# haoheliu/voicefixer

Measured on AMD Instinct MI355X. Metric: seconds-of-44.1kHz-audio restored per wall-second, higher is better.
Workload: dtype f32

## Files before the change

voicefixer_amd/csrc/vfx_conv.hip:

```cpp
#include "vfx_common.h"
#include <cstdio>
#include <cstdlib>
#include <cstring>
#include <map>
#include <mutex>
#include <string>
#include <type_traits>
#include <vector>

#ifndef VFX_X3_ABL
#define VFX_X3_ABL 0
#endif
#ifndef VFX_ABL
#define VFX_ABL 0
#endif
#define VFX_MAXPH 8
#define VFX_MAXT 9

typedef float f32x16 __attribute__((ext_vector_type(16)));
typedef unsigned int u32x4 __attribute__((ext_vector_type(4)));

#if VFX_ABL & 8
__device__ unsigned long long g_dbg[10];
__device__ unsigned long long g_dbgx[6];
// ... 906 lines not shown
        static const bool dump = VFX_DEV_ENV("VFX_DEBUG_ARGS") && atoi(VFX_DEV_ENV("VFX_DEBUG_ARGS")) != 0;
        if (dump) {
            fprintf(stderr, "conv table:");
            const unsigned* w = reinterpret_cast<const unsigned*>(&tb);
            for (size_t i = 0; i < sizeof(PhaseTab) / 4; ++i) fprintf(stderr, " %08x", w[i]);
            fprintf(stderr, "\n");
        }
    }
    ConvTables* d = nullptr;
    if (hipMalloc((void**)&d, sizeof(ConvTables)) != hipSuccess) return nullptr;
    if (hipMemcpy(d, &tb, sizeof(ConvTables), hipMemcpyHostToDevice) != hipSuccess) return nullptr;
    cache.emplace(std::move(key), d);
    return d;
}

static thread_local int g_last_tile = 0;
extern "C" int vfx_last_conv_tile(void) { return g_last_tile; }

static inline int floor4(int v) { return v >= 0 ? (v & ~3) : -(((-v) + 3) & ~3); }

template <int BM, int BL, int WGM, int WGL, int KC, bool FAST, int NXV = 4, bool SPLITK = false>
static int launch_one(const ConvArgs& a, dim3 grid, size_t lds, hipStream_t s) {
    static unsigned long long attr_set = 0;
    int attr_dev = 0;
    if (hipGetDevice(&attr_dev) != hipSuccess) attr_dev = 0;
    auto kern = conv_taps_kernel<BM, BL, WGM, WGL, KC, FAST, NXV, SPLITK>;
    if (!((attr_set >> (attr_dev & 63)) & 1ull)) {
        hipError_t e = hipFuncSetAttribute(reinterpret_cast<const void*>(kern),
                                           hipFuncAttributeMaxDynamicSharedMemorySize, 160 * 1024);
        if (e != hipSuccess) return (int)e;
        attr_set |= 1ull << (attr_dev & 63);
    }
    {
        static const bool dump = VFX_DEV_ENV("VFX_DEBUG_ARGS") && atoi(VFX_DEV_ENV("VFX_DEBUG_ARGS")) != 0;
        if (dump) {
            fprintf(stderr, "conv_taps<%d,%d,%d,%d,%d,%d,%d,%d> grid %u %u %u lds %zu args:", BM, BL, WGM, WGL, KC, (int)FAST,
                    NXV, (int)SPLITK, grid.x, grid.y, grid.z, lds);
            const unsigned* w = reinterpret_cast<const unsigned*>(&a);
            for (size_t i = 0; i < sizeof(ConvArgs) / 4; ++i) fprintf(stderr, " %08x", w[i]);
            fprintf(stderr, "\n");
        }
    }
    hipLaunchKernelGGL(kern, grid, dim3(64 * WGM * WGL), lds, s, a);
    VFX_LAUNCHED();
    return vfx_last_error();
}

template <int BM, int BL, int WGM, int WGL, int KC>
static int launch_cfg(const ConvArgs& a, int ntiles, int gy, int gz, size_t lds, hipStream_t s) {
    const int nfast = a.tile_hi - a.tile_lo;
    int rc = VFX_OK;
    if (a.ksplit > 1) {
        if (nfast > 0) rc = launch_one<BM, BL, WGM, WGL, KC, true, 4, true>(a, dim3(nfast, gy, gz), lds, s);
        if (rc == VFX_OK && ntiles - nfast > 0)
            rc = launch_one<BM, BL, WGM, WGL, KC, false, 4, true>(a, dim3(ntiles - nfast, gy, gz), lds, s);
        return rc;
    }
    if (nfast > 0) {
        const dim3 grid((nfast + a.tpw - 1) / a.tpw, gy, gz);
        if constexpr (WGM * WGL == 4) {
            rc = a.nxv <= 1   ? launch_one<BM, BL, WGM, WGL, KC, true, 1>(a, grid, lds, s)
                 : a.nxv == 2 ? launch_one<BM, BL, WGM, WGL, KC, true, 2>(a, grid, lds, s)
                 : a.nxv == 3 ? launch_one<BM, BL, WGM, WGL, KC, true, 3>(a, grid, lds, s)
                              : launch_one<BM, BL, WGM, WGL, KC, true, 4>(a, grid, lds, s);
        } else {
            rc = launch_one<BM, BL, WGM, WGL, KC, true, 4>(a, grid, lds, s);
        }
    }
    if (rc == VFX_OK && ntiles - nfast > 0)
        rc = launch_one<BM, BL, WGM, WGL, KC, false>(a, dim3(ntiles - nfast, gy, gz), lds, s);
    return rc;
}

static int fill_segments(ConvArgs& a, ConvTables& tb, int nphase, const PhaseSpec* phs, int BL, int KC,
                         bool exact = false) {
    int segw = 0;
    bool halo[VFX_MAXPH];
    for (int p = 0; p < nphase; ++p) {
        int mn = phs[p].taps[0].off, mx = mn;
        for (int t = 1; t < phs[p].ntaps; ++t) {
            mn = phs[p].taps[t].off < mn ? phs[p].taps[t].off : mn;
            mx = phs[p].taps[t].off > mx ? phs[p].taps[t].off : mx;
        }
        const int span = mx - mn;
        halo[p] = (long long)BL + span + 3 <= (long long)phs[p].ntaps * (BL + 3);
        int need;
        if (halo[p]) {
            need = exact ? BL : (mn - floor4(mn)) + BL + span;
        } else {
            need = exact ? BL : BL + 3;
        }
        need = (need + 3) & ~3;
        segw = need > segw ? need : segw;
    }
    a.segw = segw;
    int xs = 0;
    for (int p = 0; p < nphase; ++p) {
        PhaseTab& T = tb.ph[p];
        T.ntaps = phs[p].ntaps;
        T.ooff = phs[p].ooff;
        if (halo[p]) {
            int mn = phs[p].taps[0].off;
            for (int t = 1; t < phs[p].ntaps; ++t) mn = phs[p].taps[t].off < mn ? phs[p].taps[t].off : mn;
            const int org = exact ? mn : floor4(mn);
            T.nseg = 1;
            T.seg_org[0] = org;
            for (int t = 0; t < phs[p].ntaps; ++t) {
                T.tap_lds[t] = phs[p].taps[t].off - org;
                T.tap_w[t] = phs[p].taps[t].slab;
            }
        } else {
            T.nseg = phs[p].ntaps;
            for (int t = 0; t < phs[p].ntaps; ++t) {
                const int org = exact ? phs[p].taps[t].off : floor4(phs[p].taps[t].off);
                T.seg_org[t] = org;
                T.tap_lds[t] = t * KC * segw + (phs[p].taps[t].off - org);
                T.tap_w[t] = phs[p].taps[t].slab;
            }
        }
        const int fl = T.nseg * KC * segw;
        xs = fl > xs ? fl : xs;
    }
    a.xs_floats = xs;
    return VFX_OK;
}



static float* splitk_workspace(hipStream_t s, size_t bytes) {
    static std::mutex mu;
    static std::map<std::pair<int, hipStream_t>, std::pair<float*, size_t>> pool;
    int dev = 0;
    if (hipGetDevice(&dev) != hipSuccess) return nullptr;
    std::lock_guard<std::mutex> lock(mu);
    auto& e = pool[std::make_pair(dev, s)];
    if (e.second < bytes) {
        static std::vector<float*> retired;
        if (e.first) retired.push_back(e.first);
        e.first = nullptr;
        e.second = 0;
        const size_t want = bytes + bytes / 2;
        if (hipMalloc((void**)&e.first, want) != hipSuccess) { e.first = nullptr; return nullptr; }
        e.second = want;
    }
    return e.first;
}


#include "vfx_convw.inc"
#include "vfx_convwg.inc"
#include "vfx_convwg4p.inc"
#include "vfx_convwg4x.inc"
#include "vfx_convtw.inc"
#include "vfx_convwg2d.inc"
#include "vfx_resblk4.inc"
#include "vfx_resblk4s.inc"
#include "vfx_convh.inc"

template <int BM, int BL, int WGM, int WGL, int NT, int MODE, int ROWS = 1>
static int launch_x3_one(const ConvArgs& a, dim3 grid, size_t lds, hipStream_t s) {
    static unsigned long long attr_set = 0;
    int attr_dev = 0;
    if (hipGetDevice(&attr_dev) != hipSuccess) attr_dev = 0;
    auto kern = conv_x3_kernel<BM, BL, WGM, WGL, NT, MODE, ROWS>;
    if (!((attr_set >> (attr_dev & 63)) & 1ull)) {
        hipError_t e = hipFuncSetAttribute(reinterpret_cast<const void*>(kern),
                                           hipFuncAttributeMaxDynamicSharedMemorySize, 160 * 1024);
        if (e != hipSuccess) return (int)e;
        attr_set |= 1ull << (attr_dev & 63);
    }
    hipLaunchKernelGGL(kern, grid, dim3(256), lds, s, a);
    VFX_LAUNCHED();
    return vfx_last_error();
}

template <int BM, int BL, int WGM, int WGL>
static int launch_x3_tile(const ConvArgs& a, int nt, int mode, int rows, dim3 grid, size_t lds, hipStream_t s) {
    if (rows == 3 && nt == 3) return launch_x3_one<BM, BL, WGM, WGL, 3, 0, 3>(a, grid, lds, s);
    if (rows == 3) return launch_x3_one<BM, BL, WGM, WGL, 1, 0, 3>(a, grid, lds, s);
#define VFX_X3(NT_)                                                                                  \
    if (nt == NT_)                                                                                   \
        return mode == 2   ? launch_x3_one<BM, BL, WGM, WGL, NT_, 2>(a, grid, lds, s)                \
               : mode == 1 ? launch_x3_one<BM, BL, WGM, WGL, NT_, 1>(a, grid, lds, s)                \
                           : launch_x3_one<BM, BL, WGM, WGL, NT_, 0>(a, grid, lds, s);
    VFX_X3(1)
    VFX_X3(2)
    VFX_X3(3)
#undef VFX_X3
    return VFX_ENOTSUP;
}

static int try_launch_x3(ConvArgs a, const vfx_tensor* x, int nphase, const PhaseSpec* phs_in, const void* w3,
                         hipStream_t stream) {
    const int Cin = a.Cin, Cout = a.Cout, B = a.B, Lq = a.Lq, Lin = a.Lin;
    if (!w3 || !vfx_aligned16(w3) || Cin % 32 != 0 || Cout % 32 != 0) return VFX_ENOTSUP;
    if (a.pad_mode == VFX_PAD_REFLECT || a.x_rows) return VFX_ENOTSUP;
    if (((long long)a.CinPad * x->cstride + Lin + 2 * x->guard) * 4 >= (1ll << 31) - (1ll << 20)) return VFX_ENOTSUP;
    int rows = 1, P = 0;
    PhaseSpec row_spec;
    const PhaseSpec* phs = phs_in;
    if (nphase == 1 && phs_in[0].ntaps == 9) {
        P = phs_in[0].taps[3].off - phs_in[0].taps[0].off;
        for (int t = 0; t < 9; ++t)
            if (phs_in[0].taps[t].off != (t / 3 - 1) * P + (t % 3 - 1) || phs_in[0].taps[t].slab != t) return VFX_ENOTSUP;
        if (P < 4) return VFX_ENOTSUP;
        rows = 3;
        row_spec.ntaps = 3;
        row_spec.ooff = phs_in[0].ooff;
        for (int t = 0; t < 3; ++t) { row_spec.taps[t].off = t - 1; row_spec.taps[t].slab = t; }
        phs = &row_spec;
    }
    int wrow_slabs = 3;
    static const bool tapsplit_all = VFX_DEV_ENV("VFX_X3_TAPSPLIT") && atoi(VFX_DEV_ENV("VFX_X3_TAPSPLIT")) != 0;
    if (rows == 1 && nphase == 1 && phs[0].ntaps == 3 && phs[0].taps[0].slab == 0 && phs[0].taps[1].slab == 1 &&
        phs[0].taps[2].slab == 2 && phs[0].taps[1].off == 0 && phs[0].taps[0].off == -phs[0].taps[2].off &&
        (phs[0].taps[2].off > 60 || (tapsplit_all && phs[0].taps[2].off > 0))) {
        rows = 3;
        P = phs[0].taps[2].off;
        wrow_slabs = 1;
        row_spec.ntaps = 1;
        row_spec.ooff = phs[0].ooff;
        row_spec.taps[0].off = 0;
        row_spec.taps[0].slab = 0;
        phs = &row_spec;
    }
    const int nt = phs[0].ntaps;
    if (nt < 1 || nt > 3) return VFX_ENOTSUP;
    int span = 0, seg_lo = 0x7fffffff, seg_hi = -0x7fffffff;
    for (int p = 0; p < nphase; ++p) {
        if (phs[p].ntaps != nt) return VFX_ENOTSUP;
        int mn = phs[p].taps[0].off, mx = mn;
        for (int t = 1; t < nt; ++t) {
            mn = phs[p].taps[t].off < mn ? phs[p].taps[t].off : mn;
            mx = phs[p].taps[t].off > mx ? phs[p].taps[t].off : mx;
        }
        span = mx - mn > span ? mx - mn : span;
        seg_lo = mn < seg_lo ? mn : seg_lo;
        seg_hi = mx > seg_hi ? mx : seg_hi;
    }
    const int mode = span <= 8 ? 0 : (span <= 120 ? 1 : 2);
    const bool seg = mode == 2;
    int BM, BL;
    if (Cout % 128 == 0) { BM = 128; BL = 128; }
    else if (Cout % 64 == 0) {
        static const bool bl128 = VFX_DEV_ENV("VFX_X3_BL128") && atoi(VFX_DEV_ENV("VFX_X3_BL128")) != 0;
        if (!seg && Lq >= 4096 && !bl128) { BM = 64; BL = 256; }
        else { BM = 64; BL = 128; }
    } else {
        if (seg) return VFX_ENOTSUP;
        BM = 32; BL = 256;
    }
    const int segw = mode == 1 ? BL + span : BL;
    const int bl_eff = mode == 0 ? BL - span : BL;
    ConvTables tb;
    std::memset(&tb, 0, sizeof(tb));
    for (int p = 0; p < nphase; ++p) {
        PhaseTab& T = tb.ph[p];
        T.ntaps = nt;
        T.ooff = phs[p].ooff;
        int mn = phs[p].taps[0].off;
        for (int t = 1; t < nt; ++t) mn = phs[p].taps[t].off < mn ? phs[p].taps[t].off : mn;
        T.nseg = seg ? nt : 1;
        for (int t = 0; t < nt; ++t) {
            if (seg) { T.seg_org[t] = phs[p].taps[t].off; T.tap_lds[t] = t * segw; }
            else { T.seg_org[0] = mn; T.tap_lds[t] = phs[p].taps[t].off - mn; }
            T.tap_w[t] = phs[p].taps[t].slab;
        }
    }
    const int ntiles = (Lq + bl_eff - 1) / bl_eff;
    const long long g = a.x_guard;
    const int rowspan = rows == 3 ? P : 0;
    if (-(long long)seg_lo + rowspan > g) return VFX_ENOTSUP;
    if ((long long)(ntiles - 1) * bl_eff + seg_hi + BL + rowspan > (long long)Lin + g) return VFX_ENOTSUP;
    a.tab3 = device_tables(tb);
    if (!a.tab3) return VFX_EINVAL;
    const int nchunks = Cin / 16;
    a.w3 = w3;
    a.segw3 = segw;
    a.bl3 = bl_eff;
    a.xrow3 = P * 4;
    a.wrow3 = wrow_slabs * nchunks * (4 * Cout * 16);
    a.xplane3 = (seg ? nt : 1) * segw * 32;
    a.buf3 = 2 * a.xplane3 + nt * 2 * BM * 32;
    a.tile_lo = 0;
    a.tile_hi = ntiles;
    const size_t lds = 2ull * a.buf3 + (a.pre_act == VFX_PRE_AFFINE_LRELU ? (size_t)Cin * 8 : 0);
    if (lds > 160 * 1024) return VFX_ENOTSUP;
    if ((long long)ntiles * (nphase * Cout / BM) * B <= 96 && Cin * (rows == 3 && nt == 3 ? 9 : nt) >= 1024)
        return VFX_ENOTSUP;
    const dim3 grid(ntiles, nphase * Cout / BM, B);
    g_last_tile = BM * 100000 + BL * 100 + 16;
    (void)x;
    if (BM == 128) return launch_x3_tile<128, 128, 2, 2>(a, nt, mode, rows, grid, lds, stream);
    if (BM == 32) {
        if (rows == 3 && nt == 3) return launch_x3_one<32, 256, 1, 4, 3, 0, 3>(a, grid, lds, stream);
        if (rows == 3) return VFX_ENOTSUP;
        if (nt == 1 && mode == 0) return launch_x3_one<32, 256, 1, 4, 1, 0, 1>(a, grid, lds, stream);
        return VFX_ENOTSUP;
    }
    if (BL == 256) return launch_x3_tile<64, 256, 1, 4>(a, nt, mode, rows, grid, lds, stream);
    return launch_x3_tile<64, 128, 1, 4>(a, nt, mode, rows, grid, lds, stream);
}

static int launch_conv(const vfx_tensor* x, const float* w, const float* bias, const vfx_tensor* res,
                       const vfx_tensor* y, int B, int Cin, int Cout, int Lin, int Lq, int Lout,
                       int nphase, const PhaseSpec* phs, int q_shift, int q_mask, int o_rs, int o_cs,
                       int pad_mode, const vfx_act* act, int in_mask, int out_mask, hipStream_t stream) {
    if (!x || !y || !w || !x->ptr || !y->ptr || B <= 0 || Cin <= 0 || Cout <= 0 || Lin <= 0 || Lq <= 0)
        return VFX_EINVAL;
    if (Cout % 32 != 0 || nphase < 1 || nphase > VFX_MAXPH) return VFX_EINVAL;
    if (x->lstride != 1 || (x->cstride & 3) || (x->bstride & 3) || !vfx_aligned16(x->ptr) || !vfx_aligned16(w))
        return VFX_EALIGN;
    if (pad_mode == VFX_PAD_REFLECT && Lin < 8) return VFX_EINVAL;
    if (B > 65535) return VFX_EINVAL;

    ConvArgs a;
    std::memset(&a, 0, sizeof(a));
    a.x = (const float*)x->ptr;
    a.w = w;
    a.bias = bias;
    a.res = res ? (const float*)res->ptr : nullptr;
    a.y = (float*)y->ptr;
    a.B = B; a.Cin = Cin; a.CinPad = (Cin + 7) & ~7; a.Cout = Cout;
    a.Lin = Lin; a.Lq = Lq; a.Lout = Lout;
    a.x_bs = x->bstride; a.x_cs = x->cstride;
    a.x_guard = (x->guard > 0 && pad_mode != VFX_PAD_REFLECT) ? (int)x->guard : 0;
    a.x_rows = x->rows;
    a.lq_extra = Lq - Lin;
    a.y_bs = y->bstride; a.y_cs = y->cstride; a.y_ls = y->lstride;
    if (res) { a.r_bs = res->bstride; a.r_cs = res->cstride; a.r_ls = res->lstride; }
    a.q_shift = q_shift; a.q_mask = q_mask; a.o_rs = o_rs; a.o_cs = o_cs;
    a.res_init = res && nphase == 1 && q_shift == 31 && o_rs == 0 && o_cs == 1 && phs[0].ooff == 0 && Lq <= Lout &&
                 (long long)Cout * res->cstride + (long long)Lq * res->lstride < (1ll << 31);
    a.pad_mode = pad_mode;
    a.pre_act = act ? act->pre_act : VFX_PRE_NONE;
    a.pre_slope = act ? act->pre_slope : 0.f;
    a.pre_scale = act ? act->pre_scale : nullptr;
    a.pre_shift = act ? act->pre_shift : nullptr;
    a.post_act = act ? act->post_act : VFX_POST_NONE;
    a.post_slope = act ? act->post_slope : 0.f;
    if (a.pre_act == VFX_PRE_AFFINE_LRELU && (!a.pre_scale || !a.pre_shift)) return VFX_EINVAL;
    a.in_mask = in_mask; a.out_mask = out_mask;

    int maxnt = 0;
    for (int p = 0; p < nphase; ++p) maxnt = phs[p].ntaps > maxnt ? phs[p].ntaps : maxnt;
    if (maxnt < 1 || maxnt > VFX_MAXT) return VFX_EINVAL;
    if (act && act->math == VFX_MATH_BF16X3) {
        const int rc3 = try_launch_x3(a, x, nphase, phs, act->w_x3, stream);
        if (rc3 != VFX_ENOTSUP) return rc3;
    }
    if (act && act->w_wino4) {
        int rc4 = VFX_ENOTSUP;
        if (nphase == 1 && phs[0].ntaps == 9 && in_mask > 0) {
            const int P = in_mask + 1;
            bool ok = true;
            for (int t = 0; t < 9; ++t) ok &= phs[0].taps[t].off == (t / 3 - 1) * P + (t % 3 - 1) && phs[0].taps[t].slab == t;
            if (ok) rc4 = try_launch_convwg4s_2d(a, x, P, act->w_wino4, stream);
        } else {
            rc4 = try_launch_convwg4(a, x, nphase, phs, act->w_wino4, stream);
        }
        if (rc4 != VFX_ENOTSUP) return rc4;
    }
    if (act && act->w_direct) {
        int rcw = VFX_ENOTSUP;
        if (nphase == 1 && phs[0].ntaps == 9 && in_mask > 0) {
            const int P = in_mask + 1;
            bool ok = true;
            for (int t = 0; t < 9; ++t) ok &= phs[0].taps[t].off == (t / 3 - 1) * P + (t % 3 - 1) && phs[0].taps[t].slab == t;
            if (ok) rcw = try_launch_convw_2d(a, x, P, act->w_direct, stream);
        } else {
            rcw = try_launch_convw(a, x, nphase, phs, act->w_direct, stream);
        }
        if (rcw != VFX_ENOTSUP) return rcw;
    }
    int best = -1;
    float best_score = -1.f;
    for (int i = 0; i < kNumTiles; ++i) {
        const TileCfg& t = kTiles[i];
        if (Cout % t.BM) continue;
        const long long lt = (Lq + t.BL - 1) / t.BL;
        const long long nwg = lt * (long long)(nphase * Cout / t.BM) * B;
        const float tail = (float)Lq / (float)(lt * t.BL);
        const long long slots = 512;
        const float quant = (float)nwg / (float)(((nwg + slots - 1) / slots) * slots);
        const float score = t.util * tail * quant;
        if (score > best_score * 1.02f) { best_score = score; best = i; }
    }
    if (best < 0) return VFX_EINVAL;
    const TileCfg& tc = kTiles[best];

    static const bool waves8_env = VFX_DEV_ENV("VFX_WAVES8") && atoi(VFX_DEV_ENV("VFX_WAVES8")) != 0;
    const bool waves8 = waves8_env && ((tc.BM == 128 && tc.BL == 128) || (tc.BM == 64 && tc.BL == 256));
    const int nthr = waves8 ? 512 : 256;
    static const bool kc16_env = VFX_DEV_ENV("VFX_KC16") && atoi(VFX_DEV_ENV("VFX_KC16")) != 0;
    int maxspan = 0;
    bool all_segments = true;
    for (int p = 0; p < nphase; ++p) {
        int mn = phs[p].taps[0].off, mx = mn;
        for (int t = 1; t < phs[p].ntaps; ++t) {
            mn = phs[p].taps[t].off < mn ? phs[p].taps[t].off : mn;
            mx = phs[p].taps[t].off > mx ? phs[p].taps[t].off : mx;
        }
        maxspan = mx - mn > maxspan ? mx - mn : maxspan;
        all_segments &= !((long long)tc.BL + (mx - mn) + 3 <= (long long)phs[p].ntaps * (tc.BL + 3));
    }
    static const int exact_off = VFX_DEV_ENV("VFX_NO_EXACT") ? atoi(VFX_DEV_ENV("VFX_NO_EXACT")) : 0;
    bool exact = exact_off != 1 && x->guard > 0 && pad_mode != VFX_PAD_REFLECT && in_mask == 0 && !waves8 &&
                 ((maxspan > 0 && maxspan <= 8) || (all_segments && exact_off != 2));
    ConvTables tb;
    int KC, ntiles;
    size_t lds;
    for (;;) {
        KC = (kc16_env && maxnt <= 3 && tc.BM == 128 && tc.BL == 128 && !waves8 && Cin % 16 == 0) ? 16 : 8;
        for (;;) {
            std::memset(&tb, 0, sizeof(tb));
            int rc = fill_segments(a, tb, nphase, phs, tc.BL, KC, exact);
            if (rc) return rc;
            int maxseg = 0;
            for (int p = 0; p < nphase; ++p) maxseg = tb.ph[p].nseg > maxseg ? tb.ph[p].nseg : maxseg;
            const bool xfit = (long long)maxseg * KC * (a.segw / 4) <= 4 * nthr;
            a.nxv = (int)(((long long)maxseg * KC * (a.segw / 4) + nthr - 1) / nthr);
            const bool wfit = (long long)maxnt * KC * tc.BM <= (KC == 16 ? 6 : (KC == 8 ? 4 : 5)) * 4 * nthr;
            if (xfit && wfit) break;
            if (KC == 4) return VFX_ERANGE;
            KC = KC == 16 ? 8 : 4;
        }
        a.ws_floats = maxnt * KC * tc.BM;
        lds = (2ull * (a.xs_floats + a.ws_floats) + 2ull * a.CinPad) * sizeof(float);
        {
            static const long pad_kb = VFX_DEV_ENV("VFX_LDS_MIN_KB") ? atol(VFX_DEV_ENV("VFX_LDS_MIN_KB")) : 0;
            if (pad_kb > 0 && lds < (size_t)pad_kb * 1024) lds = (size_t)pad_kb * 1024;
        }
        if (lds > 160 * 1024) return VFX_ERANGE;

        a.bl_step = (exact && !all_segments) ? tc.BL - maxspan : tc.BL;
        ntiles = (Lq + a.bl_step - 1) / a.bl_step;
        int seg_lo = 0x7fffffff, seg_hi = -0x7fffffff;
        for (int p = 0; p < nphase; ++p)
            for (int sg = 0; sg < tb.ph[p].nseg; ++sg) {
                seg_lo = tb.ph[p].seg_org[sg] < seg_lo ? tb.ph[p].seg_org[sg] : seg_lo;
                seg_hi = tb.ph[p].seg_org[sg] > seg_hi ? tb.ph[p].seg_org[sg] : seg_hi;
            }
        const long long g = (x->guard > 0 && pad_mode != VFX_PAD_REFLECT) ? x->guard : 0;
        const long long need_lo = -(long long)seg_lo - g;
        int tlo = need_lo > 0 ? (int)((need_lo + a.bl_step - 1) / a.bl_step) : 0;
        const long long room = (long long)Lin + g - seg_hi - a.segw;
        int thi = room >= 0 ? (int)(room / a.bl_step) + 1 : 0;
        if (thi > ntiles) thi = ntiles;
        if (tlo > thi || Cin % KC != 0) { tlo = 0; thi = 0; }
        if (((long long)a.CinPad * x->cstride + Lin + 2 * g) * 4 >= (1ll << 31) - (1ll << 20)) { tlo = 0; thi = 0; }
        if (a.x_rows && pad_mode == VFX_PAD_REFLECT) { tlo = 0; thi = 0; }
        a.tile_lo = tlo;
        a.tile_hi = thi;
        if (exact && !(tlo == 0 && thi == ntiles)) { exact = false; continue; }
        break;
    }
    a.tab = device_tables(tb);
    if (!a.tab) return VFX_EINVAL;
    g_last_tile = tc.BM * 100000 + tc.BL * 100 + KC;
    a.ksplit = 1;
    {
        static const bool splitk_off = VFX_DEV_ENV("VFX_NO_SPLITK") && atoi(VFX_DEV_ENV("VFX_NO_SPLITK")) != 0;
        const int nchunks = (Cin + KC - 1) / KC;
        const long long nwg = (long long)ntiles * (nphase * Cout / tc.BM) * B;
        const bool plain_map = nphase == 1 && q_shift == 31 && o_rs == 0 && o_cs == 1 && phs[0].ooff == 0 && Lq <= Lout;
        if (!splitk_off && plain_map && nwg <= 192 && nchunks >= 32) {
            int want = (int)(512 / nwg);
            if (want > 8) want = 8;
            if (want > nchunks / 16) want = nchunks / 16;
            if (want >= 2 && (long long)B * want <= 65535) {
                a.cpp = (nchunks + want - 1) / want;
                a.ksplit = (nchunks + a.cpp - 1) / a.cpp;
                a.ws_ls = Lq;
                a.ws = splitk_workspace(stream, (size_t)a.ksplit * B * Cout * Lq * sizeof(float));
                if (!a.ws) a.ksplit = 1;
            }
        }
    }
    {
        const long long nwg1 = (long long)(a.tile_hi - a.tile_lo) * (nphase * Cout / tc.BM) * B;
        (void)nwg1;
        a.tpw = 1;
    }
    const int gy = nphase * Cout / tc.BM;
    const int gz = B * a.ksplit;
    int rc = VFX_EINVAL;
    if (KC == 16) rc = launch_cfg<128, 128, 2, 2, 16>(a, ntiles, gy, gz, lds, stream);
#define VFX_CASE(BM_, BL_, WGM_, WGL_)                                                          \
    else if (tc.BM == BM_ && tc.BL == BL_)                                                      \
        rc = KC == 8 ? launch_cfg<BM_, BL_, WGM_, WGL_, 8>(a, ntiles, gy, gz, lds, stream)      \
                     : launch_cfg<BM_, BL_, WGM_, WGL_, 4>(a, ntiles, gy, gz, lds, stream);
    else if (waves8 && tc.BM == 128 && tc.BL == 128)
        rc = KC == 8 ? launch_cfg<128, 128, 4, 2, 8>(a, ntiles, gy, gz, lds, stream)
                     : launch_cfg<128, 128, 4, 2, 4>(a, ntiles, gy, gz, lds, stream);
    else if (waves8 && tc.BM == 64 && tc.BL == 256)
        rc = KC == 8 ? launch_cfg<64, 256, 2, 4, 8>(a, ntiles, gy, gz, lds, stream)
                     : launch_cfg<64, 256, 2, 4, 4>(a, ntiles, gy, gz, lds, stream);
    VFX_CASE(128, 128, 2, 2)
    VFX_CASE(64, 256, 1, 4)
    VFX_CASE(128, 64, 4, 1)
    VFX_CASE(32, 256, 1, 4)
    VFX_CASE(64, 64, 2, 2)
    VFX_CASE(32, 128, 1, 4)
#undef VFX_CASE
    if (rc != VFX_OK || a.ksplit == 1) return rc;
    const long long total = (long long)B * Cout * Lq;
    const int blocks = (int)((total + 255) / 256 < 4096 ? (total + 255) / 256 : 4096);
    hipLaunchKernelGGL(splitk_reduce_kernel, dim3(blocks), dim3(256), 0, stream, a.ws, a.ksplit, a.ws_ls, a.bias, a.res,
                       a.r_bs, a.r_cs, a.r_ls, a.y, a.y_bs, a.y_cs, a.y_ls, B, Cout, Lq, a.post_act, a.post_slope,
                       a.out_mask);
    VFX_LAUNCHED();
    return vfx_last_error();
}

extern "C" int vfx_conv1d_f32(const vfx_tensor* x, const float* w_packed, const float* bias,
                              const vfx_tensor* res, const vfx_tensor* y, int B, int Cin, int Cout,
                              int L, int k, int dilation, int pad_mode, const vfx_act* act,
                              vfx_stream_t stream) {
    if (k < 1 || k > VFX_MAXT || !(k & 1) || dilation < 1) return VFX_EINVAL;
    PhaseSpec ph;
    ph.ntaps = k;
    ph.ooff = 0;
    for (int t = 0; t < k; ++t) {
        ph.taps[t].off = (t - (k - 1) / 2) * dilation;
        ph.taps[t].slab = t;
    }
    return launch_conv(x, w_packed, bias, res, y, B, Cin, Cout, L, L, L, 1, &ph, 31, 0x7fffffff, 0, 1,
                       pad_mode, act, 0, 0, (hipStream_t)stream);
}

extern "C" int vfx_convtr1d_f32(const vfx_tensor* x, const float* w_packed, const float* bias,
                                const vfx_tensor* y, int B, int Cin, int Cout, int Lin, int stride,
                                const vfx_act* act, vfx_stream_t stream) {
    if (stride < 1 || stride > VFX_MAXPH) return VFX_EINVAL;
    if (act && act->w_wino4) {
        const int rc = try_launch_convtw(x, act->w_wino4, bias, y, B, Cin, Cout, Lin, stride, act, (hipStream_t)stream);
        if (rc != VFX_ENOTSUP) return rc;
    }
    const int pad = stride / 2 + stride % 2;
    PhaseSpec ph[VFX_MAXPH];
    for (int r = 0; r < stride; ++r) {
        ph[r].ntaps = 2;
        ph[r].taps[0].off = 0;
        ph[r].taps[0].slab = r;
        ph[r].taps[1].off = -1;
        ph[r].taps[1].slab = r + stride;
        ph[r].ooff = r - pad;
    }
    return launch_conv(x, w_packed, bias, nullptr, y, B, Cin, Cout, Lin, Lin + 1, stride * Lin, stride, ph,
                       31, 0x7fffffff, 0, stride, VFX_PAD_ZERO, act, 0, 0, (hipStream_t)stream);
}

extern "C" int vfx_conv2d_f32(const vfx_tensor* x, const float* w_packed, const float* bias,
                              const vfx_tensor* res, const vfx_tensor* y, int B, int Cin, int Cout, int H,
                              int pitch_log2, int ksize, const vfx_act* act, vfx_stream_t stream) {
    if ((ksize != 1 && ksize != 3) || pitch_log2 < 1 || pitch_log2 > 12 || H < 1) return VFX_EINVAL;
    const int P = 1 << pitch_log2;
    PhaseSpec ph;
    ph.ooff = 0;
    ph.ntaps = ksize * ksize;
    for (int ky = 0; ky < ksize; ++ky)
        for (int kx = 0; kx < ksize; ++kx) {
            ph.taps[ky * ksize + kx].off = (ky - ksize / 2) * P + (kx - ksize / 2);
            ph.taps[ky * ksize + kx].slab = ky * ksize + kx;
        }
    const int L = H * P;
    return launch_conv(x, w_packed, bias, res, y, B, Cin, Cout, L, L, L, 1, &ph, 31, 0x7fffffff, 0, 1,
                       VFX_PAD_ZERO, act, P - 1, P - 1, (hipStream_t)stream);
}

extern "C" int vfx_convtr2d_3x3s2_f32(const vfx_tensor* x, const float* w_packed, const vfx_tensor* y, int B,
                                      int Cin, int Cout, int h, int in_pitch_log2, const vfx_act* act,
                                      vfx_stream_t stream) {
    if (in_pitch_log2 < 1 || in_pitch_log2 > 11 || h < 1) return VFX_EINVAL;
    const int Pi = 1 << in_pitch_log2, Po = 2 * Pi;
    PhaseSpec ph[4];
    for (int py = 0; py < 2; ++py)
        for (int px = 0; px < 2; ++px) {
            PhaseSpec& p = ph[py * 2 + px];
            p.ntaps = 0;
            p.ooff = py * Po + px;
            const int nky = py == 0 ? 2 : 1, nkx = px == 0 ? 2 : 1;
            for (int iy = 0; iy < nky; ++iy)
                for (int ix = 0; ix < nkx; ++ix) {
                    const int ky = py == 0 ? 2 * iy : 1, kx = px == 0 ? 2 * ix : 1;
                    const int dy = py == 0 ? iy : 0, dx = px == 0 ? ix : 0;
                    p.taps[p.ntaps].off = -(dy * Pi + dx);
                    p.taps[p.ntaps].slab = ky * 3 + kx;
                    ++p.ntaps;
                }
        }
    const int Lin = h * Pi;
    return launch_conv(x, w_packed, nullptr, nullptr, y, B, Cin, Cout, Lin, Lin, 2 * h * Po, 4, ph,
                       in_pitch_log2, Pi - 1, 2 * Po, 2, VFX_PAD_ZERO, act, Pi - 1, Po - 1,
                       (hipStream_t)stream);
}
```

voicefixer_amd/csrc/vfx_convtw.inc:

```
template <int WGM, int WGP>
__global__ __launch_bounds__(256, 2) void convtw_kernel(const ConvArgs a) {
    static_assert(WGM * WGP == 4, "four waves");
    constexpr int KC = 16, NSTEP = KC / 2, NPL = 4;
    constexpr int BM = 32 * WGM, BT = 32 * WGP;
    constexpr int CG = 256 / BT;
    constexpr int NSLOT = KC / CG;
    constexpr int SPAN = NSTEP / NSLOT;
    constexpr int PLANE = KC * BT;
    constexpr int BUF = NPL * PLANE;
    extern __shared__ __attribute__((aligned(16))) float smem[];

    const int tid = threadIdx.x, lane = tid & 63;
    const int wave = __builtin_amdgcn_readfirstlane(tid >> 6);
    const int lo = lane & 31, hi = lane >> 5;
    const int wm = wave / WGP, wp = wave % WGP;
    const int s = a.nph_fold, gy = a.tpw;
    int lin = blockIdx.x;
    if (a.xcd_chunk > 0) lin = (lin & 7) * a.xcd_chunk + (lin >> 3);
    if (lin >= a.ntiles_l * s * gy) return;
    int phase, mblk, tile;
    if (a.tile_lo == 0) {
        tile = lin % a.ntiles_l;
        const int rest = lin / a.ntiles_l;
        phase = rest % s; mblk = rest / s;
    } else {
        phase = lin % s;
        const int rest = lin / s;
        mblk = rest % gy; tile = rest / gy;
    }
    const int b = blockIdx.z;
    const int Lrow = a.x_rows ? __builtin_amdgcn_readfirstlane(a.x_rows[b]) : a.Lin;
    const int T0 = tile * BT;
    if (3 * T0 > Lrow) return;
    const int xcs = (int)a.x_cs;
    const int S = a.Cin / KC;

    const int st = tid % BT, cg = tid / BT;
    int xvoff[4];
    {
        const int p0 = 3 * (T0 + st) - 1;
#pragma unroll
        for (int j = 0; j < 4; ++j) xvoff[j] = (p0 + j >= 0 && p0 + j < Lrow) ? (cg * xcs + p0 + j) * 4 : VFX_W_OOB;
    }
    const __amdgpu_buffer_rsrc_t xrsrc = __builtin_amdgcn_make_buffer_rsrc(
        const_cast<float*>(a.x) + (long long)b * a.x_bs, (short)0, 0x7fffffff, 0x00020000);
    float* const wbase = smem + cg * BT + st;
    float xv[NSLOT][4];
    auto x_load_part = [&](int j, int t, int s0) {
        xv[j][t] = __uint_as_float(__builtin_amdgcn_raw_buffer_load_b32(xrsrc, xvoff[t], s0 + j * CG * xcs * 4, 0));
    };
    auto x_load = [&](int chunk) {
        const int s0 = chunk * KC * xcs * 4;
#pragma unroll
        for (int j = 0; j < NSLOT; ++j)
#pragma unroll
            for (int t = 0; t < 4; ++t) x_load_part(j, t, s0);
    };
    auto x_transform = [&](int j, float (&V)[4]) {
        V[0] = xv[j][0] - xv[j][2];
        V[1] = xv[j][1] + xv[j][2];
        V[2] = xv[j][2] - xv[j][1];
        V[3] = xv[j][3] - xv[j][1];
    };

    const __amdgpu_buffer_rsrc_t wrsrc =
        __builtin_amdgcn_make_buffer_rsrc(const_cast<float*>(a.wd), (short)0, 0x7fffffff, 0x00020000);
    const int row0 = mblk * BM + wm * 32;
    const int avoff = ((row0 + lo) * 8 + 4 * hi) * 4;
    const int gstride = a.Cout * 32;
    const int pstride = (a.CinPad >> 3) * gstride;
    const int poff = phase * NPL * pstride;
    float4 aw[2][NPL];
    auto a_load_one = [&](auto set_tag, int k, int grp) {
        constexpr int SET = decltype(set_tag)::value;
        const u32x4 r = __builtin_amdgcn_raw_buffer_load_b128(wrsrc, avoff, poff + k * pstride + grp * gstride, 0);
        aw[SET][k] = make_float4(__uint_as_float(r.x), __uint_as_float(r.y), __uint_as_float(r.z), __uint_as_float(r.w));
    };
    using S0 = std::integral_constant<int, 0>;
    using S1 = std::integral_constant<int, 1>;

    const __amdgpu_buffer_rsrc_t brsrc = __builtin_amdgcn_make_buffer_rsrc(
        const_cast<float*>(a.bias ? a.bias : a.x), (short)0, 0x7fffffff, 0x00020000);
    u32x4 bq[4];
    {
        const int bvoff = a.bias ? (row0 + 4 * hi) * 4 : VFX_W_OOB;
#pragma unroll
        for (int g = 0; g < 4; ++g) bq[g] = __builtin_amdgcn_raw_buffer_load_b128(brsrc, bvoff, g * 32, 0);
    }
    x_load(0);
#pragma unroll
    for (int k = 0; k < NPL; ++k) a_load_one(S0{}, k, 0);
    __builtin_amdgcn_sched_barrier(0);

    f32x16 acc[NPL];
    const int boffs = hi * BT + wp * 32 + lo;
    f32x16 biasv;
#pragma unroll
    for (int g = 0; g < 4; ++g) {
        biasv[4 * g + 0] = __uint_as_float(bq[g].x); biasv[4 * g + 1] = __uint_as_float(bq[g].y);
        biasv[4 * g + 2] = __uint_as_float(bq[g].z); biasv[4 * g + 3] = __uint_as_float(bq[g].w);
    }
    auto mma_chunk = [&](auto first_tag, const float* xs, float* wdst, int xchunk, int agrp0) {
        constexpr bool FIRST = decltype(first_tag)::value;
        const float* bp = xs + boffs;
        const int agrp1 = min(agrp0 + 1, 2 * S - 1), agrp2 = min(agrp0 + 2, 2 * S - 1);
        float bf[NPL];
#pragma unroll
        for (int k = 0; k < NPL; ++k) bf[k] = bp[k * PLANE];
        const int xs0 = xchunk * KC * xcs * 4;
        float V[4];
#pragma unroll
        for (int u = 0; u < NSTEP; ++u) {
            const int el = u / SPAN, ph = u % SPAN;
#pragma unroll
            for (int k = 0; k < NPL; ++k) {
                if (ph == 0 && k == 0) x_transform(el, V);
                if (ph == 0) wdst[el * CG * BT + k * PLANE] = V[k];
                if (ph == SPAN / 2) x_load_part(el, k, xs0);
                if (u == 0) a_load_one(S1{}, k, agrp1);
                if (u == 4) a_load_one(S0{}, k, agrp2);
                const float4 av4 = (u < 4) ? aw[0][k] : aw[1][k];
                const int kk = u & 3;
                const float av = kk == 0 ? av4.x : (kk == 1 ? av4.y : (kk == 2 ? av4.z : av4.w));
                if (FIRST && u == 0) {
                    const f32x16 zero16 = {0.f, 0.f, 0.f, 0.f, 0.f, 0.f, 0.f, 0.f, 0.f, 0.f, 0.f, 0.f, 0.f, 0.f, 0.f, 0.f};
                    acc[k] = __builtin_amdgcn_mfma_f32_32x32x2f32(av, bf[k], k == 1 ? biasv : zero16, 0, 0, 0);
                } else {
                    acc[k] = __builtin_amdgcn_mfma_f32_32x32x2f32(av, bf[k], acc[k], 0, 0, 0);
                }
                if (u < NSTEP - 1) bf[k] = bp[k * PLANE + (u + 1) * 2 * BT];
                __builtin_amdgcn_sched_barrier(0);
            }
        }
    };
    {
#pragma unroll
        for (int j = 0; j < NSLOT; ++j) {
            float V[4];
            x_transform(j, V);
#pragma unroll
            for (int k = 0; k < NPL; ++k) wbase[j * CG * BT + k * PLANE] = V[k];
        }
        x_load(1);
        __builtin_amdgcn_sched_barrier(0);
    }
    __syncthreads();
    mma_chunk(std::true_type{}, smem, wbase + BUF, 2 < S ? 2 : S - 1, 0);
    __syncthreads();
    mma_chunk(std::false_type{}, smem + BUF, wbase, 3 < S ? 3 : S - 1, 2);
    __syncthreads();
#pragma unroll 1
    for (int c = 2; c < S; c += 2) {
        mma_chunk(std::false_type{}, smem, wbase + BUF, min(c + 2, S - 1), 2 * c);
        __syncthreads();
        mma_chunk(std::false_type{}, smem + BUF, wbase, min(c + 3, S - 1), 2 * c + 2);
        __syncthreads();
    }

    const __amdgpu_buffer_rsrc_t yrsrc = __builtin_amdgcn_make_buffer_rsrc(
        a.y + (long long)b * a.y_bs, (short)0, 0x7fffffff, 0x00020000);
    const int ycs4 = (int)a.y_cs * 4;
    const int q0 = 3 * (T0 + wp * 32 + lo);
    int yv[3];
#pragma unroll
    for (int i = 0; i < 3; ++i) {
        const int q = q0 + i;
        const int o = q * s + phase - a.w_ooff0;
        yv[i] = (q <= Lrow && o >= 0 && o < s * Lrow) ? (4 * hi * (int)a.y_cs + o) * 4 : VFX_W_OOB;
    }
#pragma unroll
    for (int r = 0; r < 16; ++r) {
        const int soff = (row0 + (r & 3) + 8 * (r >> 2)) * ycs4;
        const float p12 = acc[1][r] + acc[2][r];
        const float y0 = acc[0][r] + p12;
        const float y1 = acc[1][r] - acc[2][r];
        const float y2 = p12 + acc[3][r];
        __builtin_amdgcn_raw_buffer_store_b32(__float_as_uint(y0), yrsrc, yv[0], soff, 0);
        __builtin_amdgcn_raw_buffer_store_b32(__float_as_uint(y1), yrsrc, yv[1], soff, 0);
        __builtin_amdgcn_raw_buffer_store_b32(__float_as_uint(y2), yrsrc, yv[2], soff, 0);
    }
}

template <int WGM, int WGP>
static int launch_convtw(const ConvArgs& a, dim3 grid, size_t lds, hipStream_t s) {
    hipLaunchKernelGGL((convtw_kernel<WGM, WGP>), grid, dim3(256), lds, s, a);
    VFX_LAUNCHED();
    return vfx_last_error();
}

static int try_launch_convtw(const vfx_tensor* x, const float* w32, const float* bias, const vfx_tensor* y, int B, int Cin, int Cout,
                             int Lin, int stride, const vfx_act* act, hipStream_t stream) {
    static const bool off = VFX_DEV_ENV("VFX_CONVTW") && atoi(VFX_DEV_ENV("VFX_CONVTW")) == 0;
    if (off || !w32 || !vfx_aligned16(w32) || !x || !y || !x->ptr || !y->ptr) return VFX_ENOTSUP;
    if (act && (act->pre_act != VFX_PRE_NONE || act->post_act != VFX_POST_NONE || act->math != VFX_MATH_F32)) return VFX_ENOTSUP;
    if (Cin % 32 != 0 || Cout % 64 != 0 || B <= 0 || B > 65535 || Lin < 1 || stride < 1) return VFX_ENOTSUP;
    if (x->lstride != 1 || y->lstride != 1 || (bias && !vfx_aligned16(bias))) return VFX_ENOTSUP;
    const long long lim = (1ll << 31) - (1ll << 20);
    if (((long long)Cin * x->cstride + Lin) * 4 >= lim || ((long long)Cout * y->cstride + (long long)stride * Lin) * 4 >= lim) return VFX_ENOTSUP;
    if (4ll * stride * (Cin >> 3) * Cout * 32 >= lim) return VFX_ENOTSUP;
    const bool wide = Cout % 128 == 0;
    const int BT = wide ? 32 : 64;
    const int ntriples = (Lin + 1 + 2) / 3;
    const int ntiles = (ntriples + BT - 1) / BT;
    const int gy = Cout / (wide ? 128 : 64);
    const long long nwg = (long long)ntiles * stride * gy;
    if (nwg * B < 512 || nwg >= (1ll << 30)) return VFX_ENOTSUP;
    ConvArgs a;
    std::memset(&a, 0, sizeof(a));
    a.x = (const float*)x->ptr;
    a.wd = w32;
    a.bias = bias;
    a.y = (float*)y->ptr;
    a.B = B; a.Cin = Cin; a.CinPad = Cin; a.Cout = Cout;
    a.Lin = Lin; a.Lq = Lin + 1; a.Lout = stride * Lin;
    a.x_bs = x->bstride; a.x_cs = x->cstride;
    a.x_rows = x->rows;
    a.y_bs = y->bstride; a.y_cs = y->cstride; a.y_ls = 1;
    a.nph_fold = stride;
    a.tpw = gy;
    a.w_ooff0 = stride / 2 + stride % 2;
    a.ntiles_l = ntiles;
    a.tile_lo = 16ll * stride * Cin * Cout <= (3ll << 20) ? 1 : 0;
    if (VFX_DEV_ENV("VFX_CONVTW_ORDER")) a.tile_lo = atoi(VFX_DEV_ENV("VFX_CONVTW_ORDER")) == 0 ? 1 : 0;
    a.xcd_chunk = nwg >= 64 ? (int)((nwg + 7) / 8) : 0;
    const dim3 grid(a.xcd_chunk > 0 ? (unsigned)(8 * a.xcd_chunk) : (unsigned)nwg, 1, B);
    const size_t lds = 2ull * 4 * 16 * BT * sizeof(float);
    g_last_tile = (wide ? 128 : 64) * 100000 + 3 * BT * 100 + 83;
    return wide ? launch_convtw<4, 1>(a, grid, lds, stream) : launch_convtw<2, 2>(a, grid, lds, stream);
}
```

Measured before the change: 1615.

## Add all-phase Winograd transposed-conv kernel sharing staged input across phases

Adds a new transposed-convolution kernel in which one workgroup computes every output phase for a tile. Each wave handles one phase and row block, and all of them share a single Winograd-transformed input tile staged in LDS. Outputs are regrouped through LDS so they can be written as coalesced 128-bit stores. This is meant to avoid reloading and retransforming the input once per phase and to cut the scattered strided stores. In exchange it uses larger workgroups (up to 896 threads for stride 7), more LDS, and fewer workgroups. It also moves the argument validation ahead of the fast path.

```diff
diff --git a/voicefixer_amd/csrc/vfx_conv.hip b/voicefixer_amd/csrc/vfx_conv.hip
--- a/voicefixer_amd/csrc/vfx_conv.hip
+++ b/voicefixer_amd/csrc/vfx_conv.hip
@@ -1232,15 +1232,21 @@
     return launch_x3_tile<64, 128, 1, 4>(a, nt, mode, rows, grid, lds, stream);
 }
 
-static int launch_conv(const vfx_tensor* x, const float* w, const float* bias, const vfx_tensor* res,
-                       const vfx_tensor* y, int B, int Cin, int Cout, int Lin, int Lq, int Lout,
-                       int nphase, const PhaseSpec* phs, int q_shift, int q_mask, int o_rs, int o_cs,
-                       int pad_mode, const vfx_act* act, int in_mask, int out_mask, hipStream_t stream) {
+static int check_conv_args(const vfx_tensor* x, const float* w, const vfx_tensor* y, int B, int Cin, int Cout, int Lin, int Lq,
+                           int nphase) {
     if (!x || !y || !w || !x->ptr || !y->ptr || B <= 0 || Cin <= 0 || Cout <= 0 || Lin <= 0 || Lq <= 0)
         return VFX_EINVAL;
     if (Cout % 32 != 0 || nphase < 1 || nphase > VFX_MAXPH) return VFX_EINVAL;
     if (x->lstride != 1 || (x->cstride & 3) || (x->bstride & 3) || !vfx_aligned16(x->ptr) || !vfx_aligned16(w))
         return VFX_EALIGN;
+    return VFX_OK;
+}
+
+static int launch_conv(const vfx_tensor* x, const float* w, const float* bias, const vfx_tensor* res,
+                       const vfx_tensor* y, int B, int Cin, int Cout, int Lin, int Lq, int Lout,
+                       int nphase, const PhaseSpec* phs, int q_shift, int q_mask, int o_rs, int o_cs,
+                       int pad_mode, const vfx_act* act, int in_mask, int out_mask, hipStream_t stream) {
+    if (const int rc = check_conv_args(x, w, y, B, Cin, Cout, Lin, Lq, nphase)) return rc;
     if (pad_mode == VFX_PAD_REFLECT && Lin < 8) return VFX_EINVAL;
     if (B > 65535) return VFX_EINVAL;
 
@@ -1463,6 +1469,7 @@
                                 const vfx_tensor* y, int B, int Cin, int Cout, int Lin, int stride,
                                 const vfx_act* act, vfx_stream_t stream) {
     if (stride < 1 || stride > VFX_MAXPH) return VFX_EINVAL;
+    if (const int rc = check_conv_args(x, w_packed, y, B, Cin, Cout, Lin, Lin + 1, stride)) return rc;
     if (act && act->w_wino4) {
         const int rc = try_launch_convtw(x, act->w_wino4, bias, y, B, Cin, Cout, Lin, stride, act, (hipStream_t)stream);
         if (rc != VFX_ENOTSUP) return rc;
diff --git a/voicefixer_amd/csrc/vfx_convtw.inc b/voicefixer_amd/csrc/vfx_convtw.inc
--- a/voicefixer_amd/csrc/vfx_convtw.inc
+++ b/voicefixer_amd/csrc/vfx_convtw.inc
@@ -188,6 +188,214 @@
     return vfx_last_error();
 }
 
+template <int S, int R>
+__global__ __launch_bounds__(64 * S * R) void convtwa_kernel(const ConvArgs a) {
+    constexpr int NW = S * R, NT = 64 * NW;
+    constexpr int KC = 16, NSTEP = KC / 2, NPL = 4;
+    constexpr int BT = 32, BM = 32 * R;
+    constexpr int SW = NW >= 8 ? 8 : 4;
+    constexpr int CG = 64 * SW / BT;
+    constexpr int NSLOT = KC / CG;
+    constexpr int SPAN = NSTEP / NSLOT;
+    constexpr int PLANE = KC * BT;
+    constexpr int BUF = NPL * PLANE;
+    constexpr int OW = 3 * BT * S;
+    constexpr int OP = OW + 4;
+    constexpr int NQ = OW / 4 + 1;
+    constexpr int RP = 8 * R;
+    static_assert(NT <= 1024 && OW % 4 == 0, "geometry");
+    extern __shared__ __attribute__((aligned(16))) float smem[];
+
+    const int tid = threadIdx.x, lane = tid & 63;
+    const int wave = __builtin_amdgcn_readfirstlane(tid >> 6);
+    const int lo = lane & 31, hi = lane >> 5;
+    const int phase = wave / R, rb = wave % R;
+    const bool stager = wave < SW;
+    const int gy = a.tpw;
+    int lin = blockIdx.x;
+    if (a.xcd_chunk > 0) lin = (lin & 7) * a.xcd_chunk + (lin >> 3);
+    if (lin >= a.ntiles_l * gy) return;
+    const int tile = lin % a.ntiles_l, mblk = lin / a.ntiles_l;
+    const int b = blockIdx.z;
+    const int Lrow = a.x_rows ? __builtin_amdgcn_readfirstlane(a.x_rows[b]) : a.Lin;
+    const int T0 = tile * BT;
+    if (3 * T0 > Lrow) return;
+    const int xcs = (int)a.x_cs;
+    const int nch = a.Cin / KC;
+
+    const int st = tid % BT, cg = (tid / BT) % CG;
+    int xvoff[4];
+    {
+        const int p0 = 3 * (T0 + st) - 1;
+#pragma unroll
+        for (int j = 0; j < 4; ++j) xvoff[j] = (p0 + j >= 0 && p0 + j < Lrow) ? (cg * xcs + p0 + j) * 4 : VFX_W_OOB;
+    }
+    const __amdgpu_buffer_rsrc_t xrsrc = __builtin_amdgcn_make_buffer_rsrc(
+        const_cast<float*>(a.x) + (long long)b * a.x_bs, (short)0, 0x7fffffff, 0x00020000);
+    float* const wbase = smem + cg * BT + st;
+    float xv[NSLOT][4];
+    auto x_load_part = [&](int j, int t, int s0) {
+        xv[j][t] = __uint_as_float(__builtin_amdgcn_raw_buffer_load_b32(xrsrc, xvoff[t], s0 + j * CG * xcs * 4, 0));
+    };
+    auto x_load = [&](int chunk) {
+        const int s0 = chunk * KC * xcs * 4;
+#pragma unroll
+        for (int j = 0; j < NSLOT; ++j)
+#pragma unroll
+            for (int t = 0; t < 4; ++t) x_load_part(j, t, s0);
+    };
+    auto x_transform = [&](int j, float (&V)[4]) {
+        V[0] = xv[j][0] - xv[j][2];
+        V[1] = xv[j][1] + xv[j][2];
+        V[2] = xv[j][2] - xv[j][1];
+        V[3] = xv[j][3] - xv[j][1];
+    };
+
+    const __amdgpu_buffer_rsrc_t wrsrc =
+        __builtin_amdgcn_make_buffer_rsrc(const_cast<float*>(a.wd), (short)0, 0x7fffffff, 0x00020000);
+    const int row0 = mblk * BM + rb * 32;
+    const int avoff = ((row0 + lo) * 8 + 4 * hi) * 4;
+    const int gstride = a.Cout * 32;
+    const int pstride = (a.CinPad >> 3) * gstride;
+    const int poff = phase * NPL * pstride;
+    float4 aw[2][NPL];
+    auto a_load_one = [&](auto set_tag, int k, int grp) {
+        constexpr int SET = decltype(set_tag)::value;
+        const u32x4 r = __builtin_amdgcn_raw_buffer_load_b128(wrsrc, avoff, poff + k * pstride + grp * gstride, 0);
+        aw[SET][k] = make_float4(__uint_as_float(r.x), __uint_as_float(r.y), __uint_as_float(r.z), __uint_as_float(r.w));
+    };
+    using S0 = std::integral_constant<int, 0>;
+    using S1 = std::integral_constant<int, 1>;
+
+    const __amdgpu_buffer_rsrc_t brsrc = __builtin_amdgcn_make_buffer_rsrc(
+        const_cast<float*>(a.bias ? a.bias : a.x), (short)0, 0x7fffffff, 0x00020000);
+    u32x4 bq[4];
+    {
+        const int bvoff = a.bias ? (row0 + 4 * hi) * 4 : VFX_W_OOB;
+#pragma unroll
+        for (int g = 0; g < 4; ++g) bq[g] = __builtin_amdgcn_raw_buffer_load_b128(brsrc, bvoff, g * 32, 0);
+    }
+    if (stager) x_load(0);
+#pragma unroll
+    for (int k = 0; k < NPL; ++k) a_load_one(S0{}, k, 0);
+    __builtin_amdgcn_sched_barrier(0);
+
+    f32x16 acc[NPL];
+    const int boffs = hi * BT + lo;
+    f32x16 biasv;
+#pragma unroll
+    for (int g = 0; g < 4; ++g) {
+        biasv[4 * g + 0] = __uint_as_float(bq[g].x); biasv[4 * g + 1] = __uint_as_float(bq[g].y);
+        biasv[4 * g + 2] = __uint_as_float(bq[g].z); biasv[4 * g + 3] = __uint_as_float(bq[g].w);
+    }
+    auto mma_chunk = [&](auto first_tag, const float* xs, float* wdst, int xchunk, int agrp0) {
+        constexpr bool FIRST = decltype(first_tag)::value;
+        const float* bp = xs + boffs;
+        const int agrp1 = min(agrp0 + 1, 2 * nch - 1), agrp2 = min(agrp0 + 2, 2 * nch - 1);
+        float bf[NPL];
+#pragma unroll
+        for (int k = 0; k < NPL; ++k) bf[k] = bp[k * PLANE];
+        const int xs0 = xchunk * KC * xcs * 4;
+        float V[4];
+#pragma unroll
+        for (int u = 0; u < NSTEP; ++u) {
+            const int el = u / SPAN, ph = u % SPAN;
+#pragma unroll
+            for (int k = 0; k < NPL; ++k) {
+                if (stager) {
+                    if (ph == 0 && k == 0) x_transform(el, V);
+                    if (ph == 0) wdst[el * CG * BT + k * PLANE] = V[k];
+                    if (ph == SPAN / 2) x_load_part(el, k, xs0);
+                }
+                if (u == 0) a_load_one(S1{}, k, agrp1);
+                if (u == 4) a_load_one(S0{}, k, agrp2);
+                const float4 av4 = (u < 4) ? aw[0][k] : aw[1][k];
+                const int kk = u & 3;
+                const float av = kk == 0 ? av4.x : (kk == 1 ? av4.y : (kk == 2 ? av4.z : av4.w));
+                if (FIRST && u == 0) {
+                    const f32x16 zero16 = {0.f, 0.f, 0.f, 0.f, 0.f, 0.f, 0.f, 0.f, 0.f, 0.f, 0.f, 0.f, 0.f, 0.f, 0.f, 0.f};
+                    acc[k] = __builtin_amdgcn_mfma_f32_32x32x2f32(av, bf[k], k == 1 ? biasv : zero16, 0, 0, 0);
+                } else {
+                    acc[k] = __builtin_amdgcn_mfma_f32_32x32x2f32(av, bf[k], acc[k], 0, 0, 0);
+                }
+                if (u < NSTEP - 1) bf[k] = bp[k * PLANE + (u + 1) * 2 * BT];
+                __builtin_amdgcn_sched_barrier(0);
+            }
+        }
+    };
+    if (stager) {
+#pragma unroll
+        for (int j = 0; j < NSLOT; ++j) {
+            float V[4];
+            x_transform(j, V);
+#pragma unroll
+            for (int k = 0; k < NPL; ++k) wbase[j * CG * BT + k * PLANE] = V[k];
+        }
+        x_load(1);
+    }
+    __builtin_amdgcn_sched_barrier(0);
+    __syncthreads();
+    mma_chunk(std::true_type{}, smem, wbase + BUF, 2 < nch ? 2 : nch - 1, 0);
+    __syncthreads();
+    mma_chunk(std::false_type{}, smem + BUF, wbase, 3 < nch ? 3 : nch - 1, 2);
+    __syncthreads();
+#pragma unroll 1
+    for (int c = 2; c < nch; c += 2) {
+        mma_chunk(std::false_type{}, smem, wbase + BUF, min(c + 2, nch - 1), 2 * c);
+        __syncthreads();
+        mma_chunk(std::false_type{}, smem + BUF, wbase, min(c + 3, nch - 1), 2 * c + 2);
+        __syncthreads();
+    }
+
+    const int o0 = 3 * T0 * S - a.w_ooff0;
+    const int sh = o0 & 3, oq = o0 - sh;
+    const int olo = max(o0, 0), ohi = min(o0 + OW, S * Lrow);
+    const __amdgpu_buffer_rsrc_t yrsrc = __builtin_amdgcn_make_buffer_rsrc(
+        a.y + (long long)b * a.y_bs, (short)0, 0x7fffffff, 0x00020000);
+    const int ycs = (int)a.y_cs;
+    float* const ow = smem + (rb * 8 + 4 * hi) * OP + 3 * S * lo + phase + sh;
+#pragma unroll
+    for (int j = 0; j < 4; ++j) {
+#pragma unroll
+        for (int e = 0; e < 4; ++e) {
+            const int r = 4 * j + e;
+            const float p12 = acc[1][r] + acc[2][r];
+            ow[e * OP + 0 * S] = acc[0][r] + p12;
+            ow[e * OP + 1 * S] = acc[1][r] - acc[2][r];
+            ow[e * OP + 2 * S] = p12 + acc[3][r];
+        }
+        __syncthreads();
+#pragma unroll 1
+        for (int idx = tid; idx < RP * NQ; idx += NT) {
+            const int rr = idx / NQ, g = idx - rr * NQ;
+            const int row = mblk * BM + (rr >> 3) * 32 + 8 * j + (rr & 7);
+            const float4 v = *reinterpret_cast<const float4*>(smem + rr * OP + 4 * g);
+            const int o = oq + 4 * g;
+            const int yo = (row * ycs + o) * 4;
+            if (o >= olo && o + 4 <= ohi) {
+                u32x4 w;
+                w.x = __float_as_uint(v.x); w.y = __float_as_uint(v.y); w.z = __float_as_uint(v.z); w.w = __float_as_uint(v.w);
+                __builtin_amdgcn_raw_buffer_store_b128(w, yrsrc, yo, 0, 0);
+            } else if (o + 4 > olo && o < ohi) {
+                __builtin_amdgcn_raw_buffer_store_b32(__float_as_uint(v.x), yrsrc, (o + 0 >= olo && o + 0 < ohi) ? yo + 0 : VFX_W_OOB, 0, 0);
+                __builtin_amdgcn_raw_buffer_store_b32(__float_as_uint(v.y), yrsrc, (o + 1 >= olo && o + 1 < ohi) ? yo + 4 : VFX_W_OOB, 0, 0);
+                __builtin_amdgcn_raw_buffer_store_b32(__float_as_uint(v.z), yrsrc, (o + 2 >= olo && o + 2 < ohi) ? yo + 8 : VFX_W_OOB, 0, 0);
+                __builtin_amdgcn_raw_buffer_store_b32(__float_as_uint(v.w), yrsrc, (o + 3 >= olo && o + 3 < ohi) ? yo + 12 : VFX_W_OOB, 0, 0);
+            }
+        }
+        if (j < 3) __syncthreads();
+    }
+}
+
+template <int S, int R>
+static int launch_convtwa(const ConvArgs& a, dim3 grid, hipStream_t s) {
+    constexpr int OP = 3 * 32 * S + 4;
+    const size_t lds = std::max<size_t>(2ull * 4 * 16 * 32, 8ull * R * OP) * sizeof(float);
+    hipLaunchKernelGGL((convtwa_kernel<S, R>), grid, dim3(64 * S * R), lds, s, a);
+    VFX_LAUNCHED();
+    return vfx_last_error();
+}
+
 static int try_launch_convtw(const vfx_tensor* x, const float* w32, const float* bias, const vfx_tensor* y, int B, int Cin, int Cout,
                              int Lin, int stride, const vfx_act* act, hipStream_t stream) {
     static const bool off = VFX_DEV_ENV("VFX_CONVTW") && atoi(VFX_DEV_ENV("VFX_CONVTW")) == 0;
@@ -200,6 +408,9 @@
     if (4ll * stride * (Cin >> 3) * Cout * 32 >= lim) return VFX_ENOTSUP;
     const bool wide = Cout % 128 == 0;
     const int BT = wide ? 32 : 64;
+    static const bool allphase_off = VFX_DEV_ENV("VFX_CONVTW_ALLPHASE") && atoi(VFX_DEV_ENV("VFX_CONVTW_ALLPHASE")) == 0;
+    const bool allphase = !allphase_off && (stride == 2 || stride == 3 || stride == 7) && vfx_aligned16(y->ptr) &&
+                          (y->cstride & 3) == 0 && (y->bstride & 3) == 0;
     const int ntriples = (Lin + 1 + 2) / 3;
     const int ntiles = (ntriples + BT - 1) / BT;
     const int gy = Cout / (wide ? 128 : 64);
@@ -222,6 +433,20 @@
     a.ntiles_l = ntiles;
     a.tile_lo = 16ll * stride * Cin * Cout <= (3ll << 20) ? 1 : 0;
     if (VFX_DEV_ENV("VFX_CONVTW_ORDER")) a.tile_lo = atoi(VFX_DEV_ENV("VFX_CONVTW_ORDER")) == 0 ? 1 : 0;
+    if (allphase) {
+        const int R = stride == 7 ? 2 : (Cout % 128 == 0 ? 4 : 2);
+        const int BM = 32 * R;
+        const int ntiles_a = (ntriples + 31) / 32;
+        const long long nwga = (long long)ntiles_a * (Cout / BM);
+        a.ntiles_l = ntiles_a;
+        a.tpw = Cout / BM;
+        a.xcd_chunk = nwga >= 64 ? (int)((nwga + 7) / 8) : 0;
+        const dim3 grid(a.xcd_chunk > 0 ? (unsigned)(8 * a.xcd_chunk) : (unsigned)nwga, 1, B);
+        g_last_tile = 1000000000 + stride * 10000000 + BM * 10000 + 96 * 100 + 83;
+        if (stride == 7) return launch_convtwa<7, 2>(a, grid, stream);
+        if (stride == 3) return R == 4 ? launch_convtwa<3, 4>(a, grid, stream) : launch_convtwa<3, 2>(a, grid, stream);
+        return R == 4 ? launch_convtwa<2, 4>(a, grid, stream) : launch_convtwa<2, 2>(a, grid, stream);
+    }
     a.xcd_chunk = nwg >= 64 ? (int)((nwg + 7) / 8) : 0;
     const dim3 grid(a.xcd_chunk > 0 ? (unsigned)(8 * a.xcd_chunk) : (unsigned)nwg, 1, B);
     const size_t lds = 2ull * 4 * 16 * BT * sizeof(float);
```

New measurement: 1610, median of 2. About the same (-0.3%).
